# CDACHPCIE25/PPQSFLHE

Hardware: AMD Instinct MI355X
Metric: ciphertexts/sec aggregated+PRE at N=2^16, L=12 RNS limbs (higher is better)
Workload: dtype u64

## Files before the change

### ppqsflhe_amd/csrc/engine.hip

```cpp
#include "engine.hpp"
#include "comm.hpp"
#include "ntt_radix.hpp"
#include "qsum_kernels.hpp"
#include "fanout_kernels.hpp"
#include "codec_kernels.hpp"
#include "sampler_kernels.hpp"

#include <cmath>
#include <cstdio>
#include <type_traits>
#include <cstdlib>
#include <cstring>

namespace mk {


template <bool INV>
__global__ __launch_bounds__(NTT_THREADS) void k_ntt_col(NttIo io, NttTables T, const u64 *scale,
                                                         const u64 *scale_sh) {
    extern __shared__ __attribute__((aligned(16))) u64 lds[];
    const uint32_t poly = blockIdx.y / io.nslots, s = blockIdx.y % io.nslots;
    if (ntt_slot_skipped(io, poly, io.vslot0 + s)) return;
    const uint32_t id = limb_id_of(io.vslot0 + s, io.nl, T.L);
    const LimbConst lc = T.limb[id];
// ... 1341 lines not shown
        NttIo s5{til, pc, (size_t)ext * n, (size_t)K * n, nl, 0, nl, K, nl};
        ntt_passes(s5, tabs_, cnt, true, fold, fold + D, lanes(), 0);
        launch_baseconv(pc, (size_t)K * n, conv, (size_t)nl * n, cv, d_limb_, n, cnt, 1, stream_);
        ntt_launch(conv, cnt, nl, nl, false, nullptr, nullptr);
    }
    k_moddown_tail<<<ew_grid(n, nl, cnt), EW_THREADS, 0, stream_>>>(til, conv, out, g, d_limb_, ext, pinv, pinv + nl,
                                                                 add, add_stride, out_stride, accumulate ? 1 : 0);
    MK_HIP(hipGetLastError());
}

void Engine::modup(const u64 *c1, u64 *digits, uint32_t cnt, uint32_t nl) {
    need_device();
    check_nl(nl);
    if (!cnt) return;
    const uint32_t n = ps_.n, ext = nl + ps_.K, nparts = ps_.num_parts(nl);
    u64 *coef = workspace((size_t)cnt * nl * n);
    modup_core(c1, (size_t)nl * n, coef, digits, cnt, nl);
    const size_t dstride = (size_t)nparts * ext * n;
    for (uint32_t part = 0; part < nparts; ++part) {
        const uint32_t lo = part * ps_.alpha, hi = std::min(nl, lo + ps_.alpha);
        k_copy_slots<<<ew_grid(n, hi - lo, cnt), EW_THREADS, 0, stream_>>>(c1, (size_t)nl * n, lo,
                                                                         digits + (size_t)part * ext * n, dstride, lo, n);
    }
    MK_HIP(hipGetLastError());
}

void Engine::moddown(const u64 *in, u64 *out, uint32_t cnt, uint32_t nl) {
    need_device();
    check_nl(nl);
    if (!cnt) return;
    const uint32_t n = ps_.n, K = ps_.K;
    const size_t w_pc = (size_t)cnt * K * n, w_conv = (size_t)cnt * nl * n;
    u64 *ws = workspace(w_pc + w_conv);
    moddown_core(in, ws, ws + w_pc, out, (size_t)nl * n, nullptr, 0, cnt, nl, false);
}

template <int NPARTS>
static void launch_inner(const u64 *dig, const u64 *c1, size_t c1_stride, const u64 *evk, u64 *til, EwGeom g,
                         const LimbConst *limb, uint32_t ext, uint32_t D, uint32_t alpha, uint32_t items,
                         unsigned long long slot_mask, hipStream_t s) {
    const uint32_t nsel = (uint32_t)__builtin_popcountll(slot_mask);
    if (!nsel) return;
    k_inner_product_b<NPARTS><<<dim3((g.n / 2 + EW_THREADS - 1) / EW_THREADS, nsel), EW_THREADS, 0, s>>>(
        dig, c1, c1_stride, evk, til, g, limb, ext, D, alpha, items, slot_mask);
}

template <int LOG_H, int NPARTS>
static void launch_row_inner_fp(const InnerArgs &a, const NttTables &T, hipStream_t s) {
    const uint32_t tiles = (1u << T.log_r1) / (256u >> LOG_H);
    const dim3 grid(tiles * a.nsel * a.items);
    k_row_inner_fp<LOG_H, NPARTS, 2><<<grid, NTT_THREADS, 0, s>>>(a, T);
}
template <int LOG_H>
static void launch_row_inner_fp_n(const InnerArgs &a, const NttTables &T, uint32_t nparts, hipStream_t s) {
    switch (nparts) {
        case 1: launch_row_inner_fp<LOG_H, 1>(a, T, s); break;
        case 2: launch_row_inner_fp<LOG_H, 2>(a, T, s); break;
        case 3: launch_row_inner_fp<LOG_H, 3>(a, T, s); break;
        case 4: launch_row_inner_fp<LOG_H, 4>(a, T, s); break;
        case 5: launch_row_inner_fp<LOG_H, 5>(a, T, s); break;
        case 6: launch_row_inner_fp<LOG_H, 6>(a, T, s); break;
        default: throw std::invalid_argument("more than 6 key-switch digits unsupported");
    }
}


template <int LOGC>
static void launch_row3_inner_fp_n(const InnerArgs &a, const NttTables &T, uint32_t nparts, hipStream_t s) {
    const dim3 grid(((1u << T.log_r1) / RowT<LOGC>::ROWS) * a.nsel * a.items);
    switch (nparts) {
        case 1: k_row3_inner_fp<1, LOGC><<<grid, NTT_THREADS, 0, s>>>(a, T); break;
        case 2: k_row3_inner_fp<2, LOGC><<<grid, NTT_THREADS, 0, s>>>(a, T); break;
        case 3: k_row3_inner_fp<3, LOGC><<<grid, NTT_THREADS, 0, s>>>(a, T); break;
        case 4: k_row3_inner_fp<4, LOGC><<<grid, NTT_THREADS, 0, s>>>(a, T); break;
        case 5: k_row3_inner_fp<5, LOGC><<<grid, NTT_THREADS, 0, s>>>(a, T); break;
        case 6: k_row3_inner_fp<6, LOGC><<<grid, NTT_THREADS, 0, s>>>(a, T); break;
        default: throw std::invalid_argument("more than 6 key-switch digits unsupported");
    }
}

template <int LOGC, bool INVP>
static void launch_row3_inner_int_k(const InnerArgs &a, const NttTables &T, uint32_t nparts, uint32_t L, u64 *pc,
                                    uint32_t K, hipStream_t s) {
    if (!a.nsel) return;
    const dim3 grid(((1u << T.log_r1) / RowT<LOGC>::ROWS) * a.nsel * a.items);
    switch (nparts) {
        case 1: with_int_arith(T, [&](auto ar) {
            k_row3_inner_int<1, LOGC, INVP, decltype(ar)::value>
                <<<grid, NTT_THREADS, 0, s>>>(a, T, L, pc, K);
        }); break;
        case 2: with_int_arith(T, [&](auto ar) {
            k_row3_inner_int<2, LOGC, INVP, decltype(ar)::value>
                <<<grid, NTT_THREADS, 0, s>>>(a, T, L, pc, K);
        }); break;
        case 3: with_int_arith(T, [&](auto ar) {
            k_row3_inner_int<3, LOGC, INVP, decltype(ar)::value>
                <<<grid, NTT_THREADS, 0, s>>>(a, T, L, pc, K);
        }); break;
        case 4: with_int_arith(T, [&](auto ar) {
            k_row3_inner_int<4, LOGC, INVP, decltype(ar)::value>
                <<<grid, NTT_THREADS, 0, s>>>(a, T, L, pc, K);
        }); break;
        case 5: with_int_arith(T, [&](auto ar) {
            k_row3_inner_int<5, LOGC, INVP, decltype(ar)::value>
                <<<grid, NTT_THREADS, 0, s>>>(a, T, L, pc, K);
        }); break;
        case 6: with_int_arith(T, [&](auto ar) {
            k_row3_inner_int<6, LOGC, INVP, decltype(ar)::value>
                <<<grid, NTT_THREADS, 0, s>>>(a, T, L, pc, K);
        }); break;
        default: throw std::invalid_argument("more than 6 key-switch digits unsupported");
    }
}
template <int LOGC>
static void launch_row3_inner_int_n(const InnerArgs &a, const NttTables &T, uint32_t nparts, uint32_t L, u64 *pc,
                                    uint32_t K, hipStream_t s) {
    if (!pc) {
        launch_row3_inner_int_k<LOGC, false>(a, T, nparts, L, nullptr, K, s);
        return;
    }
    const unsigned long long q_slots = a.nl >= 64 ? ~0ull : ((1ull << a.nl) - 1);
    InnerArgs aq = a, ap = a;
    aq.slot_mask = a.slot_mask & q_slots;
    ap.slot_mask = a.slot_mask & ~q_slots;
    aq.nsel = (uint32_t)__builtin_popcountll(aq.slot_mask);
    ap.nsel = (uint32_t)__builtin_popcountll(ap.slot_mask);
    launch_row3_inner_int_k<LOGC, true>(ap, T, nparts, L, pc, K, s);
    launch_row3_inner_int_k<LOGC, false>(aq, T, nparts, L, nullptr, K, s);
}

bool Engine::keyswitch_digits(const u64 *c1, size_t ct_stride, const u64 *evk, u64 *coef, u64 *dig, u64 *til, u64 *pc,
                              uint32_t cnt, uint32_t nl) {
    const uint32_t ext = nl + ps_.K, nparts = ps_.num_parts(nl), D = ps_.D;
    const int row_h = fast_row(tabs_.log_r2, 1u << tabs_.log_r1);
    unsigned long long fp_mask = 0, all_mask = ext >= 64 ? ~0ull : ((1ull << ext) - 1);
    for (uint32_t i = 0; i < nl; ++i)
        if (tabs_.h_fp_of[i]) fp_mask |= 1ull << i;
    bool p_fp = false;
    for (uint32_t k = 0; k < ps_.K; ++k)
        if (tabs_.h_fp_of[ps_.L + k]) p_fp = true;
    const bool fuse = fp_mask != 0 && !p_fp && (row_h == 3 || row_h == 4 || row_h == 9) &&
                      fast_log_h(tabs_.log_r1, 1u << tabs_.log_r2) != 0;
    const bool fuse_int = fuse && (row_h == 4 || row_h == 9);
    {
        struct Reset {
            bool &flag;
            ~Reset() { flag = false; }
        } reset{skip_rows_};
        skip_rows_ = fuse_int;
        modup_core(c1, ct_stride, coef, dig, cnt, nl, fuse);
    }
    if (fuse) {
        InnerArgs a{dig, c1, evk, til, ct_stride, nl, ext, D, ps_.alpha, cnt, fp_mask,
                    (uint32_t)__builtin_popcountll(fp_mask)};
        if (row_h == 9) launch_row3_inner_fp_n<3>(a, tabs_, nparts, stream_);
        else if (row_h == 4) launch_row_inner_fp_n<4>(a, tabs_, nparts, stream_);
        else launch_row_inner_fp_n<3>(a, tabs_, nparts, stream_);
    }
    const unsigned long long mask = fuse ? (all_mask & ~fp_mask) : all_mask;
    if (fuse_int) {
        InnerArgs a{dig, c1, evk, til, ct_stride, nl, ext, D, ps_.alpha, cnt, mask, (uint32_t)__builtin_popcountll(mask)};
        u64 *pc_fused = pc;
        if (row_h == 9) launch_row3_inner_int_n<3>(a, tabs_, nparts, ps_.L, pc_fused, ps_.K, stream_);
        else launch_row3_inner_int_n<2>(a, tabs_, nparts, ps_.L, pc_fused, ps_.K, stream_);
        MK_HIP(hipGetLastError());
        return pc_fused != nullptr;
    }
    inner_product_all(c1, ct_stride, evk, dig, til, cnt, nl, mask);
// ... 789 lines not shown
```

### ppqsflhe_amd/csrc/ntt_radix.hpp

```cpp
#pragma once
#include "modarith.hpp"
#include "ntt_kernels.hpp"

namespace mk {

#ifndef MK_NT8
#define MK_NT8 0
#endif
MK_D u64 ld_stream(const u64 *p) { return (MK_NT && MK_NT8) ? __builtin_nontemporal_load(p) : *p; }
MK_D ulong2 ld_stream2(const ulong2 *p) {
    if (MK_NT) {
        ulong2 v;
        v.x = __builtin_nontemporal_load(&p->x);
        v.y = __builtin_nontemporal_load(&p->y);
        return v;
    }
    return *p;
}
MK_D u64 ld_pass(const u64 *p) { return (MK_NT >= 2 && MK_NT8) ? __builtin_nontemporal_load(p) : *p; }
#ifndef MK_NT8S
#define MK_NT8S 1
#endif
MK_D void st_pass(u64 *p, u64 v) {
    if (MK_NT >= 2 && MK_NT8S) __builtin_nontemporal_store(v, p);
    else *p = v;
}
MK_D ulong2 ld_pass2(const ulong2 *p) {
    if (MK_NT >= 2) {
        ulong2 v;
        v.x = __builtin_nontemporal_load(&p->x);
        v.y = __builtin_nontemporal_load(&p->y);
        return v;
    }
    return *p;
}
MK_D void st_pass2(ulong2 *p, ulong2 v) {
    if (MK_NT >= 2) {
        __builtin_nontemporal_store(v.x, &p->x);
        __builtin_nontemporal_store(v.y, &p->y);
    } else {
        *p = v;
    }
}
MK_D void st_stream2(ulong2 *p, ulong2 v) {
    if (MK_NT) {
        __builtin_nontemporal_store(v.x, &p->x);
        __builtin_nontemporal_store(v.y, &p->y);
    } else {
        *p = v;
    }
}

#ifndef MK_STAMP
#define MK_STAMP 0
#endif
constexpr unsigned STAMP_REGION = 1u << 20, STAMP_REGIONS = 4;
struct Stamper {
    unsigned long long t[8];
    MK_D Stamper() {
#pragma unroll
        for (int i = 0; i < 8; ++i) t[i] = 0;
    }
    template <int K>
    MK_D void mark() {
        if (MK_STAMP) {
            __builtin_amdgcn_sched_barrier(0);
            t[K] = __builtin_amdgcn_s_memtime();
            __builtin_amdgcn_sched_barrier(0);
        }
    }
    template <int K>
    MK_D unsigned long long add(unsigned long long since) {
        if (MK_STAMP) {
            __builtin_amdgcn_sched_barrier(0);
            const unsigned long long now = __builtin_amdgcn_s_memtime();
            __builtin_amdgcn_sched_barrier(0);
            t[K] += now - since;
            return now;
        }
        return 0;
    }
    MK_D unsigned long long now() {
        if (MK_STAMP) {
            __builtin_amdgcn_sched_barrier(0);
            const unsigned long long v = __builtin_amdgcn_s_memtime();
            __builtin_amdgcn_sched_barrier(0);
            return v;
        }
        return 0;
    }
    template <int REGION>
    MK_D void flush(unsigned long long *buf, bool differences) {
        if (MK_STAMP && buf && (threadIdx.x & 63) == 0) {
            const unsigned b = blockIdx.x + gridDim.x * (blockIdx.y + gridDim.y * blockIdx.z);
            unsigned long long *p = buf + (size_t)REGION * STAMP_REGION + ((b * 4 + threadIdx.x / 64) % (STAMP_REGION / 8)) * 8;
#pragma unroll
            for (int i = 0; i < 8; ++i) p[i] = differences ? (i + 1 < 8 && t[i + 1] ? t[i + 1] - t[i] : 0) : t[i];
        }
    }
};

MK_D void group_member(uint32_t b, uint32_t groups, uint32_t members, uint32_t cu_affine, uint32_t &grp, uint32_t &mem) {
    if (groups % 8 == 0) {
        const uint32_t xcd = b % 8, qidx = b / 8;
        if (cu_affine && groups % 256 == 0) {
            const uint32_t per = 32 * members, blk = qidx / per, r = qidx % per;
            grp = (blk * 32 + r % 32) * 8 + xcd;
            mem = r / 32;
        } else {
            grp = (qidx / members) * 8 + xcd;
            mem = qidx % members;
        }
    } else {
        grp = b / members;
        mem = b % members;
    }
}

MK_D void conv_item_tile(uint32_t grp, uint32_t groups, uint32_t items, uint32_t tiles, uint32_t &item, uint32_t &tile) {
    if (groups % 8 == 0 && items % 8 == 0) {
        const uint32_t u = grp / 8;
        tile = u % tiles;
        item = (u / tiles) * 8 + grp % 8;
    } else {
        item = grp / tiles;
        tile = grp % tiles;
    }
}

template <int LOG_H>
MK_D void load_round_twiddles(const u64 *__restrict__ tw, const u64 *__restrict__ tw_sh, uint32_t base_eff,
                              u64 (&w)[(1 << LOG_H) - 1], u64 (&wp)[(1 << LOG_H) - 1]) {
#pragma unroll
    for (int s = 0; s < LOG_H; ++s) {
        const uint32_t first = base_eff << s;
#pragma unroll
        for (int g = 0; g < (1 << s); ++g) {
            w[(1 << s) - 1 + g] = tw[first + g];
            wp[(1 << s) - 1 + g] = tw_sh[first + g];
        }
    }
}

template <int LOG_H>
MK_D void load_rowb_twiddles(const u64 *__restrict__ twb_limb, uint32_t row, int j, u64 (&w)[(1 << LOG_H) - 1],
                             u64 (&wp)[(1 << LOG_H) - 1]) {
    constexpr int H = 1 << LOG_H;
    const ulong2 *p = reinterpret_cast<const ulong2 *>(twb_limb) + (size_t)row * H * H + j;
#pragma unroll
    for (int i = 0; i < H - 1; ++i) {
        const ulong2 t = p[i * H];
        w[i] = t.x;
        wp[i] = t.y;
    }
}

template <int LOG_H>
MK_D void radix_forward(u64 (&x)[1 << LOG_H], const u64 (&w)[(1 << LOG_H) - 1], const u64 (&wp)[(1 << LOG_H) - 1],
                        u64 q, u64 q2) {
    constexpr int H = 1 << LOG_H;
    const u64 q4 = q2 + q2;
#pragma unroll
    for (int s = 0; s < LOG_H; ++s) {
        const int dist = H >> (s + 1);
#pragma unroll
        for (int p = 0; p < H / 2; ++p) {
            const int g = p / dist, k0 = g * 2 * dist + (p % dist);
            if (s % 2 == 0) ct_butterfly_c4(x[k0], x[k0 + dist], w[(1 << s) - 1 + g], wp[(1 << s) - 1 + g], q, q2, q4);
            else ct_butterfly_nc(x[k0], x[k0 + dist], w[(1 << s) - 1 + g], wp[(1 << s) - 1 + g], q, q2);
        }
    }
}
// ... 1504 lines not shown
                zy += zz.y;
            }
            if ((cl & 7) == 7) {
                tx = reduce_word(tx, lc);
                ty = reduce_word(ty, lc);
                zx = reduce_word(zx, lc);
                zy = reduce_word(zy, lc);
            }
        }
        tx = reduce_word(tx, lc);
        ty = reduce_word(ty, lc);
        ulong2 v;
        v.x = shoup_mul(sub_mod(tx, lds[TL::at(c.g, xx)], lc.q), pi, pi_sh, lc.q);
        v.y = shoup_mul(sub_mod(ty, lds[TL::at(c.g, xx + 1)], lc.q), pi, pi_sh, lc.q);
        if (with_c0) {
            v.x = add_mod(v.x, reduce_word(zx, lc), lc.q);
            v.y = add_mod(v.y, reduce_word(zy, lc), lc.q);
        }
        if (a.init_from_out) {
            const ulong2 o = reinterpret_cast<const ulong2 *>(dst)[e];
            v.x = add_mod(v.x, o.x, lc.q);
            v.y = add_mod(v.y, o.y, lc.q);
        }
        reinterpret_cast<ulong2 *>(dst)[e] = v;
    }
}

template <int LOGC, int AR>
MK_D void row3_inverse_int(u64 (&x)[8], const Row3Ctx &c, const u64 (&wc)[7], const u64 (&wpc)[7], const LimbConst &lc) {
    using TL = RowT<LOGC>;
    constexpr int S = TL::ROWS, TPR = TL::TPR, C = TL::C;
    const int a = c.t / C, cc = c.t % C;
    if (LOGC == 3) {
        radix_inverse_any<3, AR>(x, wc, wpc, lc);
    } else {
        u64 y0[4] = {x[0], x[1], x[2], x[3]}, y1[4] = {x[4], x[5], x[6], x[7]};
        const u64 w0[3] = {wc[0], wc[1], wc[2]}, wp0[3] = {wpc[0], wpc[1], wpc[2]};
        const u64 w1[3] = {wc[3], wc[4], wc[5]}, wp1[3] = {wpc[3], wpc[4], wpc[5]};
        radix_inverse_any<2, AR>(y0, w0, wp0, lc);
        radix_inverse_any<2, AR>(y1, w1, wp1, lc);
#pragma unroll
        for (int k = 0; k < 4; ++k) {
            x[k] = y0[k];
            x[4 + k] = y1[k];
        }
    }
#pragma unroll
    for (int k = 0; k < 8; ++k) c.lds[TL::at(c.g, 8 * c.t + k)] = x[k];
    wave_lds_sync();
#pragma unroll
    for (int k = 0; k < 8; ++k) x[k] = c.lds[TL::at(c.g, 8 * C * a + C * k + cc)];
    u64 w[7], wp[7];
#pragma unroll
    for (int s = 0; s < 3; ++s)
#pragma unroll
        for (int gg = 0; gg < (1 << s); ++gg) {
            const int e = S * 8 * ((1 << s) - 1) + ((c.g * 8 + a) << s) + gg;
            w[(1 << s) - 1 + gg] = c.twb[e];
            wp[(1 << s) - 1 + gg] = c.twb_sh[e];
        }
    radix_inverse_any<3, AR>(x, w, wp, lc);
#pragma unroll
    for (int k = 0; k < 8; ++k) c.lds[TL::at(c.g, 8 * C * a + C * k + cc)] = x[k];
    wave_lds_sync();
#pragma unroll
    for (int k = 0; k < 8; ++k) x[k] = c.lds[TL::at(c.g, c.t + TPR * k)];
#pragma unroll
    for (int s = 0; s < 3; ++s)
#pragma unroll
        for (int gg = 0; gg < (1 << s); ++gg) {
            const int e = S * ((1 << s) - 1) + (c.g << s) + gg;
            w[(1 << s) - 1 + gg] = c.twa[e];
            wp[(1 << s) - 1 + gg] = c.twa_sh[e];
        }
    radix_inverse_any<3, AR>(x, w, wp, lc);
}

#ifndef MK_INVP_WAVES
#define MK_INVP_WAVES 2
#endif
#ifndef MK_INNERQ_WAVES
#define MK_INNERQ_WAVES 2
#endif
template <int NPARTS, int LOGC, bool INVP, int AR>
__global__ __launch_bounds__(NTT_THREADS, INVP ? MK_INVP_WAVES : MK_INNERQ_WAVES) void k_row3_inner_int(InnerArgs a, NttTables T, uint32_t L, u64 *pc,
                                                                   uint32_t K) {
    using TL = RowT<LOGC>;
    constexpr int R = TL::R, S = TL::ROWS, TPR = TL::TPR, PAIRS = 4;
    __shared__ u64 lds[TL::WORDS + 2 * (TL::TWA + TL::TWB)];
    Row3Ctx c;
    c.lds = lds;
    c.twa = lds + TL::WORDS;
    c.twa_sh = c.twa + TL::TWA;
    c.twb = c.twa_sh + TL::TWA;
    c.twb_sh = c.twb + TL::TWB;
    const uint32_t n = 1u << T.log_n, r1 = 1u << T.log_r1;
    const uint32_t tiles = r1 / S, groups = tiles * a.nsel;
    uint32_t grp, item;
    group_member(blockIdx.x, groups, a.items, T.cu_affine, grp, item);
    const uint32_t sl = nth_set_bit(a.slot_mask, grp / tiles);
    const uint32_t id = limb_id_of(sl, a.nl, L);
    const LimbConst lc = T.limb[id];
    const int own = sl < a.nl ? (int)(sl / a.alpha) : -1;
    const uint32_t row0 = (grp % tiles) * S;
    c.g = threadIdx.x / TPR;
    c.t = threadIdx.x % TPR;
    const u64 *tw = T.tw + (size_t)id * n, *tw_sh = T.tw_sh + (size_t)id * n;
    row3_stage_twiddles<LOGC>(c, tw, tw_sh, r1 + row0);
    u64 wc[7], wpc[7];
    row3_load_c_twiddles<LOGC>(tw, tw_sh, r1 + row0 + c.g, c.t, wc, wpc);
    const size_t tile_off = (size_t)row0 * R;
    const u64 *evk = inner_evk(a, item);
    int jn = own == 0 ? 1 : 0;
    const u64 *dig0 = a.dig + ((size_t)item * NPARTS * a.ext + sl) * n + tile_off + (size_t)c.g * R + c.t;
    u64 x[8];
    if (jn < NPARTS) {
        const u64 *src = dig0 + (size_t)jn * a.ext * n;
#pragma unroll
        for (int k = 0; k < 8; ++k) x[k] = ld_stream(src + TPR * k);
    }
    u64 h0[2 * PAIRS], l0[2 * PAIRS], h1[2 * PAIRS], l1[2 * PAIRS];
#pragma unroll
    for (int i = 0; i < 2 * PAIRS; ++i) h0[i] = l0[i] = h1[i] = l1[i] = 0;
    if (own >= 0) {
        const u64 *y0 = inner_c1(a, item) + (size_t)sl * n + tile_off;
        const u64 *e0 = evk + (((size_t)own * 2 + 0) * a.D + id) * n + tile_off;
        const u64 *e1 = evk + (((size_t)own * 2 + 1) * a.D + id) * n + tile_off;
#pragma unroll
        for (int i = 0; i < PAIRS; ++i) {
            const int e = row3_pair<LOGC>(c.g, c.t, i);
            const ulong2 yy = ld_stream2(reinterpret_cast<const ulong2 *>(y0) + e);
            const ulong2 b = reinterpret_cast<const ulong2 *>(e0)[e];
            const ulong2 cc = reinterpret_cast<const ulong2 *>(e1)[e];
            mac128(h0[2 * i], l0[2 * i], yy.x, b.x);
            mac128(h0[2 * i + 1], l0[2 * i + 1], yy.y, b.y);
            mac128(h1[2 * i], l1[2 * i], yy.x, cc.x);
            mac128(h1[2 * i + 1], l1[2 * i + 1], yy.y, cc.y);
        }
    }
    __syncthreads();
#pragma unroll 1
    for (int dj = jn; dj < NPARTS; dj = jn) {
        jn = dj + 1 == own ? dj + 2 : dj + 1;
        wave_lds_sync();
        row3_forward<AR, LOGC>(x, c, wc, wpc, lc);
#pragma unroll
        for (int k = 0; k < 8; ++k) lds[TL::at(c.g, 8 * c.t + k)] = AR == AR_PM ? x[k] : canon8(x[k], lc.q, lc.q2);
        if (jn < NPARTS) {
            const u64 *src = dig0 + (size_t)jn * a.ext * n;
#pragma unroll
            for (int k = 0; k < 8; ++k) x[k] = ld_stream(src + TPR * k);
        }
        wave_lds_sync();
        const u64 *e0 = evk + (((size_t)dj * 2 + 0) * a.D + id) * n + tile_off;
        const u64 *e1 = evk + (((size_t)dj * 2 + 1) * a.D + id) * n + tile_off;
        ulong2 eb[PAIRS], ec[PAIRS];
        constexpr bool BURST = INVP ? MK_INVP_WAVES == 2 : MK_INNERQ_WAVES == 2;
        if (BURST) {
#pragma unroll
            for (int i = 0; i < PAIRS; ++i) {
                const int e = row3_pair<LOGC>(c.g, c.t, i);
                eb[i] = reinterpret_cast<const ulong2 *>(e0)[e];
                ec[i] = reinterpret_cast<const ulong2 *>(e1)[e];
            }
            __builtin_amdgcn_sched_barrier(0);
        }
#pragma unroll
        for (int i = 0; i < PAIRS; ++i) {
            const int e = row3_pair<LOGC>(c.g, c.t, i);
            const int xx = (2 * e) % R;
            const ulong2 b = BURST ? eb[i] : reinterpret_cast<const ulong2 *>(e0)[e];
            const ulong2 cc = BURST ? ec[i] : reinterpret_cast<const ulong2 *>(e1)[e];
            const u64 yx = lds[TL::at(c.g, xx)], yz = lds[TL::at(c.g, xx + 1)];
            mac128(h0[2 * i], l0[2 * i], yx, b.x);
            mac128(h0[2 * i + 1], l0[2 * i + 1], yz, b.y);
            mac128(h1[2 * i], l1[2 * i], yx, cc.x);
            mac128(h1[2 * i + 1], l1[2 * i + 1], yz, cc.y);
        }
    }
    constexpr bool inv = INVP;
    const u64 *itw = T.itw + (size_t)id * n, *itw_sh = T.itw_sh + (size_t)id * n;
    if (inv) {
        __syncthreads();
        row3_stage_twiddles<LOGC>(c, itw, itw_sh, r1 + row0);
        __syncthreads();
    }
#pragma unroll 1
    for (int comp = 0; comp < 2; ++comp) {
        ulong2 res[PAIRS];
#pragma unroll
        for (int i = 0; i < PAIRS; ++i) {
            const u64 hx = comp ? h1[2 * i] : h0[2 * i], lx = comp ? l1[2 * i] : l0[2 * i];
            const u64 hy = comp ? h1[2 * i + 1] : h0[2 * i + 1], ly = comp ? l1[2 * i + 1] : l0[2 * i + 1];
            if (AR == AR_PM) {
                const PmK P = pm_consts(lc);
                res[i].x = pm_reduce128(hx, lx, P, lc.q);
                res[i].y = pm_reduce128(hy, ly, P, lc.q);
            } else {
                res[i].x = NPARTS <= 4 ? reduce_sum4(hx, lx, lc) : reduce_wide(hx, lx, lc);
                res[i].y = NPARTS <= 4 ? reduce_sum4(hy, ly, lc) : reduce_wide(hy, ly, lc);
            }
        }
        if (!inv) {
            u64 *td = a.til + (a.til_compact ? ((size_t)item * 2 + comp) * a.nsel + grp / tiles
                                             : ((size_t)item * 2 + comp) * a.ext + sl) * n + tile_off;
#pragma unroll
            for (int i = 0; i < PAIRS; ++i) st_stream2(reinterpret_cast<ulong2 *>(td) + row3_pair<LOGC>(c.g, c.t, i), res[i]);
        } else {
            wave_lds_sync();
#pragma unroll
            for (int i = 0; i < PAIRS; ++i) {
                const int xx = (2 * row3_pair<LOGC>(c.g, c.t, i)) % R;
                lds[TL::at(c.g, xx)] = res[i].x;
                lds[TL::at(c.g, xx + 1)] = res[i].y;
            }
            wave_lds_sync();
#pragma unroll
            for (int k = 0; k < 8; ++k) x[k] = lds[TL::at(c.g, 8 * c.t + k)];
            u64 iwc[7], iwpc[7];
            row3_load_c_twiddles<LOGC>(itw, itw_sh, r1 + row0 + c.g, c.t, iwc, iwpc);
            row3_inverse_int<LOGC, AR>(x, c, iwc, iwpc, lc);
            u64 *pd = pc + (((size_t)item * 2 + comp) * K + (sl - a.nl)) * n + tile_off + (size_t)c.g * R + c.t;
#pragma unroll
            for (int k = 0; k < 8; ++k) st_pass(pd + TPR * k, x[k]);
        }
    }
}


MK_D u64 lift_signed(int64_t v, const LimbConst &lc) {
    const u64 m = reduce_word(v < 0 ? (u64)0 - (u64)v : (u64)v, lc);
    return (v < 0 && m != 0) ? lc.q - m : m;
}
MK_D u64 lift_signed(int8_t v, const LimbConst &lc) { return v == 0 ? 0 : (v > 0 ? 1 : lc.q - 1); }

struct LiftIo {
    const int8_t *v;
    const int64_t *e0, *e1;
    u64 *out;
    uint32_t nl;
    unsigned long long slot_mask;
    uint32_t nsel;
};

template <int LOG_H, int AR>
__global__ __launch_bounds__(NTT_THREADS, 4) void k_lift_col(LiftIo io, NttTables T) {
    using TL = ColTile<LOG_H>;
    constexpr int H = TL::H, S = TL::S;
    __shared__ u64 lds[TL::WORDS + ColTwB<LOG_H>::WORDS];
    const uint32_t n = 1u << T.log_n, r2 = 1u << T.log_r2;
    const uint32_t which = blockIdx.y / io.nsel, sl = nth_set_bit(io.slot_mask, blockIdx.y % io.nsel), item = blockIdx.z;
    const LimbConst lc = T.limb[sl];
    if ((lc.fp != 0) != (AR == AR_FP)) return;
    const int c = threadIdx.x % S, j = threadIdx.x / S;
    const size_t s0 = (size_t)item * n + blockIdx.x * S + c;
    u64 x[H];
    if (which == 0) {
#pragma unroll
        for (int k = 0; k < H; ++k) x[k] = lift_signed(io.v[s0 + (size_t)(j + H * k) * r2], lc);
    } else {
        const int64_t *e = (which == 1 ? io.e0 : io.e1) + s0;
#pragma unroll
        for (int k = 0; k < H; ++k) x[k] = lift_signed(e[(size_t)(j + H * k) * r2], lc);
    }
    if (AR == AR_FP) {
#pragma unroll
        for (int k = 0; k < H; ++k) x[k] = dbits(u52_to_double(x[k]));
    }
    u64 *dst = io.out + (((size_t)item * 3 + which) * io.nl + sl) * n + blockIdx.x * S + c;
    col_forward_finish<LOG_H, AR>(x, lds, T.tw + (size_t)sl * n, T.tw_sh + (size_t)sl * n, lc, j, c, dst, r2);
}

struct RerandArgs {
    const u64 *col;
    const u64 *ct;
    const u64 *pk;
    u64 *out;
    uint32_t nl_in, nl, D;
    unsigned long long slot_mask;
    uint32_t nsel;
};

template <int LOG_H, int AR>
MK_D void rerand_row_forward(const u64 *src, u64 *lds, const u64 *twa, const u64 *twa_sh, const u64 *twb, uint32_t row0,
                             int g, int j, const LimbConst &lc) {
    using TL = RowTile<LOG_H>;
    constexpr int H = TL::H, R = TL::R;
    u64 x[H], w[H - 1], wp[H - 1];
#pragma unroll
    for (int k = 0; k < H; ++k) x[k] = ld_pass(src + (size_t)g * R + j + H * k);
    RowTwA<LOG_H>::fetch(twa, twa_sh, g, w, wp);
    radix_forward_any<LOG_H, AR>(x, w, wp, lc);
    load_rowb_twiddles<LOG_H>(twb, row0 + g, j, w, wp);
    wave_lds_sync();
#pragma unroll
    for (int k = 0; k < H; ++k) lds[TL::at(g, j + H * k)] = x[k];
    wave_lds_sync();
#pragma unroll
    for (int k = 0; k < H; ++k) x[k] = lds[TL::at(g, H * j + k)];
    radix_forward_any<LOG_H, AR>(x, w, wp, lc);
#pragma unroll
    for (int k = 0; k < H; ++k)
        lds[TL::at(g, H * j + k)] = (AR == AR_FP) ? fp_to_canonical(bitsd(x[k]), lc.qd, lc.qinv) : canon8(x[k], lc.q, lc.q2);
    wave_lds_sync();
}

#ifndef MK_RERAND_VLDS
#define MK_RERAND_VLDS 1
#endif
// ... 179 lines not shown
```

Before: 31730.

## Walk multiple items per block in key-switch inner kernel to reuse staged twiddles

Each block of the row3 inner-product kernel now processes a walk of up to MK_INNER_WALK items that share the same limb tile. Twiddles are staged into LDS once per block instead of once per item. For the inverse path, the inverse twiddles and per-column twiddles are staged into a separate LDS region up front rather than restaged after a barrier. A new block-to-(group,walk) mapping keeps CU/XCD affinity, and timing stamps are added behind MK_STAMP. The launch grid shrinks accordingly. The trade-off is more LDS use, a longer serial loop per block with fewer blocks in flight, and reloading column twiddles on each item in the lean path.

```diff
diff --git a/ppqsflhe_amd/csrc/engine.hip b/ppqsflhe_amd/csrc/engine.hip
--- a/ppqsflhe_amd/csrc/engine.hip
+++ b/ppqsflhe_amd/csrc/engine.hip
@@ -1447,8 +1447,8 @@
 template <int LOGC, bool INVP>
 static void launch_row3_inner_int_k(const InnerArgs &a, const NttTables &T, uint32_t nparts, uint32_t L, u64 *pc,
                                     uint32_t K, hipStream_t s) {
-    if (!a.nsel) return;
-    const dim3 grid(((1u << T.log_r1) / RowT<LOGC>::ROWS) * a.nsel * a.items);
+    if (!a.nsel || !a.items) return;
+    const dim3 grid(((1u << T.log_r1) / RowT<LOGC>::ROWS) * a.nsel * inner_walks(a, nparts));
     switch (nparts) {
         case 1: with_int_arith(T, [&](auto ar) {
             k_row3_inner_int<1, LOGC, INVP, decltype(ar)::value>
diff --git a/ppqsflhe_amd/csrc/ntt_radix.hpp b/ppqsflhe_amd/csrc/ntt_radix.hpp
--- a/ppqsflhe_amd/csrc/ntt_radix.hpp
+++ b/ppqsflhe_amd/csrc/ntt_radix.hpp
@@ -54,7 +54,7 @@
 #ifndef MK_STAMP
 #define MK_STAMP 0
 #endif
-constexpr unsigned STAMP_REGION = 1u << 20, STAMP_REGIONS = 4;
+constexpr unsigned STAMP_REGION = 1u << 20, STAMP_REGIONS = 5;
 struct Stamper {
     unsigned long long t[8];
     MK_D Stamper() {
@@ -88,6 +88,9 @@
             return v;
         }
         return 0;
+    }
+    MK_D void drain_vm() {
+        if (MK_STAMP) __builtin_amdgcn_s_waitcnt(0x0F70);
     }
     template <int REGION>
     MK_D void flush(unsigned long long *buf, bool differences) {
@@ -1758,12 +1761,38 @@
 #ifndef MK_INNERQ_WAVES
 #define MK_INNERQ_WAVES 2
 #endif
+#ifndef MK_INNER_WALK
+#define MK_INNER_WALK 4
+#endif
+MK_HD constexpr uint32_t inner_walk_len(uint32_t nparts) { return nparts == 1 ? 1 : MK_INNER_WALK; }
+MK_HD uint32_t inner_walk_ipc(const InnerArgs &a) { return a.ipc < a.items ? a.ipc : a.items; }
+MK_HD uint32_t inner_walks(const InnerArgs &a, uint32_t nparts) {
+    const uint32_t ipc = inner_walk_ipc(a), w = inner_walk_len(nparts);
+    return ipc ? (a.items / ipc) * ((ipc + w - 1) / w) : 0;
+}
+MK_D void walk_member(uint32_t b, uint32_t groups, uint32_t members, uint32_t cu_affine, uint32_t &grp, uint32_t &mem) {
+    if (cu_affine && groups % 8 == 0 && groups % 256 != 0) {
+        const uint32_t gx = groups / 8, low = gx & (0u - gx), cc = low < 32 ? low : 32, lanes = 32 / cc;
+        if (members % lanes == 0) {
+            const uint32_t xcd = b % 8, qidx = b / 8, per = cc * members;
+            const uint32_t blk = qidx / per, r = qidx % per, col = r % 32;
+            grp = (blk * cc + col % cc) * 8 + xcd;
+            mem = (r / 32) * lanes + col / cc;
+            return;
+        }
+    }
+    group_member(b, groups, members, cu_affine, grp, mem);
+}
 template <int NPARTS, int LOGC, bool INVP, int AR>
 __global__ __launch_bounds__(NTT_THREADS, INVP ? MK_INVP_WAVES : MK_INNERQ_WAVES) void k_row3_inner_int(InnerArgs a, NttTables T, uint32_t L, u64 *pc,
                                                                    uint32_t K) {
     using TL = RowT<LOGC>;
-    constexpr int R = TL::R, S = TL::ROWS, TPR = TL::TPR, PAIRS = 4;
-    __shared__ u64 lds[TL::WORDS + 2 * (TL::TWA + TL::TWB)];
+    constexpr int R = TL::R, S = TL::ROWS, TPR = TL::TPR, PAIRS = 4, W = inner_walk_len(NPARTS);
+    constexpr int TWW = 2 * (TL::TWA + TL::TWB);
+    constexpr int NC = INVP ? (LOGC == 3 ? 7 : 6) : 0;
+    constexpr bool LEAN = AR != AR_PM;
+    __shared__ u64 lds[TL::WORDS + (INVP ? 2 : 1) * TWW];
+    __shared__ ulong2 ldsc[NC ? NC * NTT_THREADS : 1];
     Row3Ctx c;
     c.lds = lds;
     c.twa = lds + TL::WORDS;
@@ -1772,8 +1801,10 @@
     c.twb_sh = c.twb + TL::TWB;
     const uint32_t n = 1u << T.log_n, r1 = 1u << T.log_r1;
     const uint32_t tiles = r1 / S, groups = tiles * a.nsel;
-    uint32_t grp, item;
-    group_member(blockIdx.x, groups, a.items, T.cu_affine, grp, item);
+    const uint32_t ipc = inner_walk_ipc(a), wper = (ipc + W - 1) / W;
+    uint32_t grp, wk;
+    walk_member(blockIdx.x, groups, inner_walks(a, NPARTS), T.cu_affine, grp, wk);
+    const uint32_t i0 = (wk % wper) * W, item0 = (wk / wper) * ipc + i0, wn = ipc - i0 < (uint32_t)W ? ipc - i0 : (uint32_t)W;
     const uint32_t sl = nth_set_bit(a.slot_mask, grp / tiles);
     const uint32_t id = limb_id_of(sl, a.nl, L);
     const LimbConst lc = T.limb[id];
@@ -1781,126 +1812,167 @@
     const uint32_t row0 = (grp % tiles) * S;
     c.g = threadIdx.x / TPR;
     c.t = threadIdx.x % TPR;
+    Row3Ctx ci = c;
+    ci.twa = c.twa + TWW;
+    ci.twa_sh = c.twa_sh + TWW;
+    ci.twb = c.twb + TWW;
+    ci.twb_sh = c.twb_sh + TWW;
+    ci.twc = ldsc;
     const u64 *tw = T.tw + (size_t)id * n, *tw_sh = T.tw_sh + (size_t)id * n;
+    Stamper stm;
+    unsigned long long t_mark = stm.now();
     row3_stage_twiddles<LOGC>(c, tw, tw_sh, r1 + row0);
     u64 wc[7], wpc[7];
-    row3_load_c_twiddles<LOGC>(tw, tw_sh, r1 + row0 + c.g, c.t, wc, wpc);
+    if (INVP) {
+        const u64 *itw = T.itw + (size_t)id * n, *itw_sh = T.itw_sh + (size_t)id * n;
+        row3_stage_twiddles<LOGC>(ci, itw, itw_sh, r1 + row0);
+        row3_load_c_twiddles<LOGC>(itw, itw_sh, r1 + row0 + c.g, c.t, wc, wpc);
+        row3_park_c_twiddles<LOGC>(ci, wc, wpc);
+    }
+    if (!LEAN) row3_load_c_twiddles<LOGC>(tw, tw_sh, r1 + row0 + c.g, c.t, wc, wpc);
     const size_t tile_off = (size_t)row0 * R;
-    const u64 *evk = inner_evk(a, item);
-    int jn = own == 0 ? 1 : 0;
-    const u64 *dig0 = a.dig + ((size_t)item * NPARTS * a.ext + sl) * n + tile_off + (size_t)c.g * R + c.t;
+    const u64 *evk0 = inner_evk(a, item0);
+    const int j0 = own == 0 ? 1 : 0;
+    const size_t dig_limb = (size_t)a.ext * n, dig_item = NPARTS * dig_limb;
+    const u64 *dig0 = a.dig + (size_t)item0 * dig_item + (size_t)sl * n + tile_off;
+    const uint32_t th = (uint32_t)c.g * R + c.t;
     u64 x[8];
-    if (jn < NPARTS) {
-        const u64 *src = dig0 + (size_t)jn * a.ext * n;
-#pragma unroll
-        for (int k = 0; k < 8; ++k) x[k] = ld_stream(src + TPR * k);
-    }
-    u64 h0[2 * PAIRS], l0[2 * PAIRS], h1[2 * PAIRS], l1[2 * PAIRS];
-#pragma unroll
-    for (int i = 0; i < 2 * PAIRS; ++i) h0[i] = l0[i] = h1[i] = l1[i] = 0;
-    if (own >= 0) {
-        const u64 *y0 = inner_c1(a, item) + (size_t)sl * n + tile_off;
-        const u64 *e0 = evk + (((size_t)own * 2 + 0) * a.D + id) * n + tile_off;
-        const u64 *e1 = evk + (((size_t)own * 2 + 1) * a.D + id) * n + tile_off;
-#pragma unroll
-        for (int i = 0; i < PAIRS; ++i) {
-            const int e = row3_pair<LOGC>(c.g, c.t, i);
-            const ulong2 yy = ld_stream2(reinterpret_cast<const ulong2 *>(y0) + e);
-            const ulong2 b = reinterpret_cast<const ulong2 *>(e0)[e];
-            const ulong2 cc = reinterpret_cast<const ulong2 *>(e1)[e];
-            mac128(h0[2 * i], l0[2 * i], yy.x, b.x);
-            mac128(h0[2 * i + 1], l0[2 * i + 1], yy.y, b.y);
-            mac128(h1[2 * i], l1[2 * i], yy.x, cc.x);
-            mac128(h1[2 * i + 1], l1[2 * i + 1], yy.y, cc.y);
-        }
+    if (!LEAN && j0 < NPARTS) {
+        const u64 *src = dig0 + j0 * dig_limb;
+#pragma unroll
+        for (int k = 0; k < 8; ++k) x[k] = ld_stream(src + th + TPR * k);
     }
     __syncthreads();
+    stm.drain_vm();
+    t_mark = stm.add<0>(t_mark);
 #pragma unroll 1
-    for (int dj = jn; dj < NPARTS; dj = jn) {
-        jn = dj + 1 == own ? dj + 2 : dj + 1;
-        wave_lds_sync();
-        row3_forward<AR, LOGC>(x, c, wc, wpc, lc);
-#pragma unroll
-        for (int k = 0; k < 8; ++k) lds[TL::at(c.g, 8 * c.t + k)] = AR == AR_PM ? x[k] : canon8(x[k], lc.q, lc.q2);
-        if (jn < NPARTS) {
-            const u64 *src = dig0 + (size_t)jn * a.ext * n;
-#pragma unroll
-            for (int k = 0; k < 8; ++k) x[k] = ld_stream(src + TPR * k);
-        }
-        wave_lds_sync();
-        const u64 *e0 = evk + (((size_t)dj * 2 + 0) * a.D + id) * n + tile_off;
-        const u64 *e1 = evk + (((size_t)dj * 2 + 1) * a.D + id) * n + tile_off;
-        ulong2 eb[PAIRS], ec[PAIRS];
-        constexpr bool BURST = INVP ? MK_INVP_WAVES == 2 : MK_INNERQ_WAVES == 2;
-        if (BURST) {
+    for (uint32_t it = 0; it < wn; ++it, dig0 += dig_item) {
+        const uint32_t item = item0 + it;
+        const u64 *evk = evk0;
+        if (LEAN) {
+            uint32_t z = 0, thl = th;
+            asm volatile("" : "+s"(z), "+v"(thl));
+            const int tl = thl % TPR, gl = thl / R;
+            evk += z;
+            row3_load_c_twiddles<LOGC>(tw + z, tw_sh + z, r1 + row0 + gl, tl, wc, wpc);
+            if (j0 < NPARTS) {
+                const u64 *src = dig0 + j0 * dig_limb;
+#pragma unroll
+                for (int k = 0; k < 8; ++k) x[k] = ld_stream(src + th + TPR * k);
+            }
+        }
+        u64 h0[2 * PAIRS], l0[2 * PAIRS], h1[2 * PAIRS], l1[2 * PAIRS];
+#pragma unroll
+        for (int i = 0; i < 2 * PAIRS; ++i) h0[i] = l0[i] = h1[i] = l1[i] = 0;
+        if (own >= 0) {
+            const u64 *y0 = inner_c1(a, item) + (size_t)sl * n + tile_off;
+            const u64 *e0 = evk + (((size_t)own * 2 + 0) * a.D + id) * n + tile_off;
+            const u64 *e1 = evk + (((size_t)own * 2 + 1) * a.D + id) * n + tile_off;
 #pragma unroll
             for (int i = 0; i < PAIRS; ++i) {
                 const int e = row3_pair<LOGC>(c.g, c.t, i);
-                eb[i] = reinterpret_cast<const ulong2 *>(e0)[e];
-                ec[i] = reinterpret_cast<const ulong2 *>(e1)[e];
-            }
-            __builtin_amdgcn_sched_barrier(0);
-        }
-#pragma unroll
-        for (int i = 0; i < PAIRS; ++i) {
-            const int e = row3_pair<LOGC>(c.g, c.t, i);
-            const int xx = (2 * e) % R;
-            const ulong2 b = BURST ? eb[i] : reinterpret_cast<const ulong2 *>(e0)[e];
-            const ulong2 cc = BURST ? ec[i] : reinterpret_cast<const ulong2 *>(e1)[e];
-            const u64 yx = lds[TL::at(c.g, xx)], yz = lds[TL::at(c.g, xx + 1)];
-            mac128(h0[2 * i], l0[2 * i], yx, b.x);
-            mac128(h0[2 * i + 1], l0[2 * i + 1], yz, b.y);
-            mac128(h1[2 * i], l1[2 * i], yx, cc.x);
-            mac128(h1[2 * i + 1], l1[2 * i + 1], yz, cc.y);
-        }
-    }
-    constexpr bool inv = INVP;
-    const u64 *itw = T.itw + (size_t)id * n, *itw_sh = T.itw_sh + (size_t)id * n;
-    if (inv) {
-        __syncthreads();
-        row3_stage_twiddles<LOGC>(c, itw, itw_sh, r1 + row0);
-        __syncthreads();
-    }
+                const ulong2 yy = ld_stream2(reinterpret_cast<const ulong2 *>(y0) + e);
+                const ulong2 b = reinterpret_cast<const ulong2 *>(e0)[e];
+                const ulong2 cc = reinterpret_cast<const ulong2 *>(e1)[e];
+                mac128(h0[2 * i], l0[2 * i], yy.x, b.x);
+                mac128(h0[2 * i + 1], l0[2 * i + 1], yy.y, b.y);
+                mac128(h1[2 * i], l1[2 * i], yy.x, cc.x);
+                mac128(h1[2 * i + 1], l1[2 * i + 1], yy.y, cc.y);
+            }
+            t_mark = stm.add<2>(t_mark);
+        }
+        int jn = j0;
 #pragma unroll 1
-    for (int comp = 0; comp < 2; ++comp) {
-        ulong2 res[PAIRS];
-#pragma unroll
-        for (int i = 0; i < PAIRS; ++i) {
-            const u64 hx = comp ? h1[2 * i] : h0[2 * i], lx = comp ? l1[2 * i] : l0[2 * i];
-            const u64 hy = comp ? h1[2 * i + 1] : h0[2 * i + 1], ly = comp ? l1[2 * i + 1] : l0[2 * i + 1];
-            if (AR == AR_PM) {
-                const PmK P = pm_consts(lc);
-                res[i].x = pm_reduce128(hx, lx, P, lc.q);
-                res[i].y = pm_reduce128(hy, ly, P, lc.q);
+        for (int dj = jn; dj < NPARTS; dj = jn) {
+            jn = dj + 1 == own ? dj + 2 : dj + 1;
+            wave_lds_sync();
+            row3_forward<AR, LOGC>(x, c, wc, wpc, lc);
+#pragma unroll
+            for (int k = 0; k < 8; ++k) lds[TL::at(c.g, 8 * c.t + k)] = AR == AR_PM ? x[k] : canon8(x[k], lc.q, lc.q2);
+            const u64 *src = jn < NPARTS ? dig0 + jn * dig_limb : (!LEAN && it + 1 < wn ? dig0 + dig_item + j0 * dig_limb : nullptr);
+            if (src) {
+#pragma unroll
+                for (int k = 0; k < 8; ++k) x[k] = ld_stream(src + th + TPR * k);
+            }
+            wave_lds_sync();
+            t_mark = stm.add<1>(t_mark);
+            const u64 *e0 = evk + (((size_t)dj * 2 + 0) * a.D + id) * n + tile_off;
+            const u64 *e1 = evk + (((size_t)dj * 2 + 1) * a.D + id) * n + tile_off;
+            ulong2 eb[PAIRS], ec[PAIRS];
+            constexpr bool BURST = INVP ? MK_INVP_WAVES == 2 : MK_INNERQ_WAVES == 2;
+            if (BURST) {
+#pragma unroll
+                for (int i = 0; i < PAIRS; ++i) {
+                    const int e = row3_pair<LOGC>(c.g, c.t, i);
+                    eb[i] = reinterpret_cast<const ulong2 *>(e0)[e];
+                    ec[i] = reinterpret_cast<const ulong2 *>(e1)[e];
+                }
+                __builtin_amdgcn_sched_barrier(0);
+            }
+#pragma unroll
+            for (int i = 0; i < PAIRS; ++i) {
+                const int e = row3_pair<LOGC>(c.g, c.t, i);
+                const int xx = (2 * e) % R;
+                const ulong2 b = BURST ? eb[i] : reinterpret_cast<const ulong2 *>(e0)[e];
+                const ulong2 cc = BURST ? ec[i] : reinterpret_cast<const ulong2 *>(e1)[e];
+                const u64 yx = lds[TL::at(c.g, xx)], yz = lds[TL::at(c.g, xx + 1)];
+                mac128(h0[2 * i], l0[2 * i], yx, b.x);
+                mac128(h0[2 * i + 1], l0[2 * i + 1], yz, b.y);
+                mac128(h1[2 * i], l1[2 * i], yx, cc.x);
+                mac128(h1[2 * i + 1], l1[2 * i + 1], yz, cc.y);
+            }
+            t_mark = stm.add<2>(t_mark);
+        }
+        constexpr bool inv = INVP;
+#pragma unroll 1
+        for (int comp = 0; comp < 2; ++comp) {
+            ulong2 res[PAIRS];
+#pragma unroll
+            for (int i = 0; i < PAIRS; ++i) {
+                const u64 hx = comp ? h1[2 * i] : h0[2 * i], lx = comp ? l1[2 * i] : l0[2 * i];
+                const u64 hy = comp ? h1[2 * i + 1] : h0[2 * i + 1], ly = comp ? l1[2 * i + 1] : l0[2 * i + 1];
+                if (AR == AR_PM) {
+                    const PmK P = pm_consts(lc);
+                    res[i].x = pm_reduce128(hx, lx, P, lc.q);
+                    res[i].y = pm_reduce128(hy, ly, P, lc.q);
+                } else {
+                    res[i].x = NPARTS <= 4 ? reduce_sum4(hx, lx, lc) : reduce_wide(hx, lx, lc);
+                    res[i].y = NPARTS <= 4 ? reduce_sum4(hy, ly, lc) : reduce_wide(hy, ly, lc);
+                }
+            }
+            t_mark = stm.add<4>(t_mark);
+            if (!inv) {
+                u64 *td = a.til + (a.til_compact ? ((size_t)item * 2 + comp) * a.nsel + grp / tiles
+                                                 : ((size_t)item * 2 + comp) * a.ext + sl) * n + tile_off;
+#pragma unroll
+                for (int i = 0; i < PAIRS; ++i) st_stream2(reinterpret_cast<ulong2 *>(td) + row3_pair<LOGC>(c.g, c.t, i), res[i]);
+                t_mark = stm.add<7>(t_mark);
             } else {
-                res[i].x = NPARTS <= 4 ? reduce_sum4(hx, lx, lc) : reduce_wide(hx, lx, lc);
-                res[i].y = NPARTS <= 4 ? reduce_sum4(hy, ly, lc) : reduce_wide(hy, ly, lc);
-            }
-        }
-        if (!inv) {
-            u64 *td = a.til + (a.til_compact ? ((size_t)item * 2 + comp) * a.nsel + grp / tiles
-                                             : ((size_t)item * 2 + comp) * a.ext + sl) * n + tile_off;
-#pragma unroll
-            for (int i = 0; i < PAIRS; ++i) st_stream2(reinterpret_cast<ulong2 *>(td) + row3_pair<LOGC>(c.g, c.t, i), res[i]);
-        } else {
-            wave_lds_sync();
-#pragma unroll
-            for (int i = 0; i < PAIRS; ++i) {
-                const int xx = (2 * row3_pair<LOGC>(c.g, c.t, i)) % R;
-                lds[TL::at(c.g, xx)] = res[i].x;
-                lds[TL::at(c.g, xx + 1)] = res[i].y;
-            }
-            wave_lds_sync();
-#pragma unroll
-            for (int k = 0; k < 8; ++k) x[k] = lds[TL::at(c.g, 8 * c.t + k)];
-            u64 iwc[7], iwpc[7];
-            row3_load_c_twiddles<LOGC>(itw, itw_sh, r1 + row0 + c.g, c.t, iwc, iwpc);
-            row3_inverse_int<LOGC, AR>(x, c, iwc, iwpc, lc);
-            u64 *pd = pc + (((size_t)item * 2 + comp) * K + (sl - a.nl)) * n + tile_off + (size_t)c.g * R + c.t;
-#pragma unroll
-            for (int k = 0; k < 8; ++k) st_pass(pd + TPR * k, x[k]);
-        }
-    }
+                wave_lds_sync();
+#pragma unroll
+                for (int i = 0; i < PAIRS; ++i) {
+                    const int xx = (2 * row3_pair<LOGC>(c.g, c.t, i)) % R;
+                    lds[TL::at(c.g, xx)] = res[i].x;
+                    lds[TL::at(c.g, xx + 1)] = res[i].y;
+                }
+                wave_lds_sync();
+                u64 y[8];
+#pragma unroll
+                for (int k = 0; k < 8; ++k) y[k] = lds[TL::at(c.g, 8 * c.t + k)];
+                u64 iwc[7], iwpc[7];
+                row3_fetch_c_twiddles<LOGC>(ci, iwc, iwpc);
+                t_mark = stm.add<5>(t_mark);
+                row3_inverse_int<LOGC, AR>(y, ci, iwc, iwpc, lc);
+                t_mark = stm.add<6>(t_mark);
+                u64 *pd = pc + (((size_t)item * 2 + comp) * K + (sl - a.nl)) * n + tile_off;
+#pragma unroll
+                for (int k = 0; k < 8; ++k) st_pass(pd + th + TPR * k, y[k]);
+                t_mark = stm.add<7>(t_mark);
+            }
+        }
+    }
+    if (INVP) stm.flush<3>(T.stamps, false);
+    else stm.flush<4>(T.stamps, false);
 }
 
 
```

New measurement: 32380 (median of 6 runs). 1.02x the previous value.
